# SandroMartens/DBGSOM

Measured on AMD Instinct MI355X. Metric: samples/sec/epoch (BMU+update), higher is better.
Workload: dtype f64; 1 GPU; Synthetic N=1e6 d=784 fp32, M=1024 (32x32); samples_total=1000000, samples_per_gpu=1000000, features=784, prototypes=1024, x_storage=f32, map=frozen (same prototypes every step), bmu_algorithm=filtered, via=HipBackend -> dbgsom_ctx_epoch (one C-ABI call per step)

## Files before the change

dbgsom_amd/backend.py:

```python
from __future__ import annotations

import ctypes
import os
from dataclasses import dataclass
from typing import Optional

import numpy as np

from . import _native


@dataclass
class EpochResult:
    new_weights: np.ndarray
    change_total: float
    errors: np.ndarray
    activations: np.ndarray
    winners: Optional[np.ndarray] = None
    distances: Optional[np.ndarray] = None
    new_weights_dev: object = None
    class_hist: Optional[np.ndarray] = None


def shard_bounds(n: int, rank: int, world: int):
# ... 293 lines not shown
                         lambda self, a: self._set("algorithm", _native.ALGORITHMS[a]))
    sweep_planes = property(lambda self: self._get("sweep_planes"),
                            lambda self, v: self._set("sweep_planes", v))
    seed_stride = property(lambda self: self._get("seed_stride"),
                           lambda self, v: self._set("seed_stride", v))
    refine = property(lambda self: self._get("refine"), lambda self, v: self._set("refine", int(v)))
    refined = property(lambda self: bool(self._get("refined")))
    defer = property(lambda self: bool(self._get("defer")), lambda self, v: self._set("defer", int(bool(v))))
    shard_smooth = property(lambda self: self._get("shard_smooth"), lambda self, v: self._set("shard_smooth", int(v)))
    shard_epochs = property(lambda self: self._get("shard_epochs"))
    defer_epochs = property(lambda self: self._get("defer_epochs"))
    csr_densify_below = property(lambda self: self._get("csr_densify_below"),
                                 lambda self, v: self._set("csr_densify_below", int(v)))
    resident_csr = property(lambda self: bool(self._get("resident_csr")))
    planes_cached = property(lambda self: bool(self._get("planes_cached")))
    padded_features = property(lambda self: self._get("padded_features"))

    @property
    def n_samples(self):
        return self._get("n_samples")

    def _require_loaded(self):
        if not self._loaded:
            raise RuntimeError("HipBackend: call load(X) first")

    def _install_collective(self):
        rank, world = dist_info()
        force = os.environ.get("DBGSOM_FORCE_COLLECTIVE") == "1" and _group_is_up()
        if world == 1 and not force:
            _native.call("dbgsom_ctx_set_collectives", self._ctx, None, None, 0, 1)
# ... 517 lines not shown
        keep, p, M, rf = self._w_arg(W)
        counts = np.empty(M, dtype=np.int64)
        win = np.empty(self._N, dtype=np.int64) if want_winners else None
        self._call("dbgsom_ctx_partition", self._ctx, p, M, rf, counts.ctypes.data,
                   None if win is None else win.ctypes.data)
        return counts, win

    def subset(self, neuron):
        child = ctypes.c_void_p()
        self._call("dbgsom_ctx_subset_create", self._ctx, int(neuron), ctypes.byref(child))
        sub = HipBackend(self.device_index, self.algorithm, _ctx=child)
        sub._weighted = self._weighted
        return sub

    _SETTABLE = ("algorithm", "sweep_planes", "seed_stride", "timing", "graph", "refine", "defer",
                 "filter_min_query_rows", "max_mean_candidates", "shard_smooth", "csr_densify_below")

    def release(self):
        if self._ctx:
            opts = {k: self._get(k) for k in self._SETTABLE}
            _native.call("dbgsom_ctx_destroy", self._ctx)
            self._ctx = ctypes.c_void_p()
            _native.call("dbgsom_ctx_create", self.device_index, ctypes.byref(self._ctx))
            for k, v in opts.items():
                self._set(k, v)
            self._install_collective()
        self._loaded = False
        self._borrowed = None
        self._hop_key = None
        self._weighted = False
        self._sw = None
# ... 9 lines not shown
```

dbgsom_amd/csrc/common.h:

```cpp
#pragma once
#include <hip/hip_runtime.h>
#include <stdint.h>
#include <stdio.h>

#include "../../include/dbgsom_hip.h"

namespace dbgsom {

void set_error(const char *fmt, ...);

#define DBGSOM_HIP_CHECK(expr)                                                           \
    do {                                                                                 \
        hipError_t _e = (expr);                                                          \
        if (_e != hipSuccess) {                                                          \
            ::dbgsom::set_error("%s failed: %s (%s:%d)", #expr, hipGetErrorString(_e),   \
                                __FILE__, __LINE__);                                     \
            return DBGSOM_EHIP;                                                          \
        }                                                                                \
    } while (0)

#define DBGSOM_REQUIRE(cond, msg)                                   \
    do {                                                            \
        if (!(cond)) {                                              \
            ::dbgsom::set_error("%s: %s", __func__, msg);           \
// ... 176 lines not shown
    const int32_t *order = nullptr;
    int seed_stride = 0, sweep_planes = 0, round_f32 = 0;
    int k = 1;
    int64_t *idx = nullptr;
    double *dist = nullptr;
    void *ws = nullptr;
    size_t ws_bytes = 0;
    hipStream_t stream = nullptr;
    const double *hint_dist = nullptr, *hint_shift = nullptr;
    int refine_rows = 0;
    bool defer_dist = false;
    const void *X_store = nullptr;
    int store_dtype = -1;
    int64_t ld_store = 0;
    double guard_mean = 0.0;
    FilterAux *aux = nullptr;
};
constexpr int DBGSOM_LISTS_LONG = 1000;
int launch_bmu_filtered(const FilteredCall &call);
size_t smooth_workspace_bytes(int64_t M, int64_t d);
int launch_smooth(const double *sums, int64_t M, int64_t d, const float *hop, double sigma,
                  int layout, const double *W_old, double *W_new, double *change_total, void *ws,
                  size_t ws_bytes, hipStream_t s);
int64_t smooth_block_cols(int64_t d, int nranks);
int64_t smooth_block_elems(int64_t M, int64_t d, int nranks);
int launch_pack_blocks(const double *sums, int64_t M, int64_t d, int nranks, double *out, hipStream_t s);
int launch_smooth_block(const double *S_b, const double *K, const double *a, int64_t M, int64_t cb, int64_t d_full,
                        const float *hop, double sigma, int layout, double *Wb, void *ws, size_t ws_bytes,
                        hipStream_t s);
int launch_rowchange_blocks(const double *blocks, int64_t M, int64_t d, int64_t cb, const double *W_old, double *W_new,
// ... 4 lines not shown
```

dbgsom_amd/csrc/engine.hip:

```cpp
#include <dlfcn.h>
#include <math.h>
#include <stdlib.h>
#include <string.h>

#include <chrono>
#include <new>
#include <vector>

#include "common.h"
#include "search_policy.h"

namespace dbgsom {

struct DevBuf {
    void *p = nullptr;
    size_t cap = 0;
    bool tight = false;
    int reserve(size_t bytes) {
        if (bytes <= cap) return DBGSOM_OK;
        if (p) { (void)hipFree(p); p = nullptr; cap = 0; }
        const size_t want = tight ? align_up(bytes) : align_up(bytes + bytes / 8, 1 << 20);
        hipError_t e = hipMalloc(&p, want);
        if (e != hipSuccess) {
            p = nullptr;
// ... 119 lines not shown
        dst[i] = src[ids[first + i]];
}
__global__ void gather_i32_kernel(const int32_t *__restrict__ src, const int32_t *__restrict__ ids, int64_t first,
                                  int64_t n, int32_t *__restrict__ dst) {
    for (int64_t i = (int64_t)blockIdx.x * blockDim.x + threadIdx.x; i < n; i += (int64_t)gridDim.x * blockDim.x)
        dst[i] = src[ids[first + i]];
}
template <typename T>
__global__ void rows_to_f64_kernel(const T *__restrict__ src, int64_t ld, const int64_t *__restrict__ ids, int64_t n,
                                   int64_t cols, double *__restrict__ dst) {
    const int64_t r = blockIdx.x;
    if (r >= n) return;
    const T *s = src + ids[r] * ld;
    for (int64_t c = threadIdx.x; c < cols; c += blockDim.x) dst[r * cols + c] = widen(s[c]);
}
__global__ void seg_counts_kernel(const uint32_t *__restrict__ seg_start, int64_t M, int64_t N, int64_t *__restrict__ counts) {
    for (int64_t j = (int64_t)blockIdx.x * blockDim.x + threadIdx.x; j < M; j += (int64_t)gridDim.x * blockDim.x)
        counts[j] = (int64_t)((j + 1 < M ? seg_start[j + 1] : (uint32_t)N) - seg_start[j]);
}

static unsigned grid1d(int64_t n, int block = 256) {
    const int64_t nb = (n + block - 1) / block;
    return (unsigned)(nb < 1 ? 1 : (nb > 8192 ? 8192 : nb));
}

}

using namespace dbgsom;

extern "C" {
const unsigned long long *dbgsom_filter_count_sum_ptr(const void *workspace_dev, int64_t N, int64_t d, int64_t M);
size_t dbgsom_filter_planes_bytes(int64_t rows, int64_t d);
size_t dbgsom_bmu_filtered_workspace_bytes(int64_t N, int64_t d, int64_t M);
}

namespace {

struct Samples {
    int dtype = -1;
    int64_t N = 0, d = 0, dp = 0;
    const void *X = nullptr;
    const void *Xb = nullptr;
    int bdtype = -1;
    DevBuf own, x32, xx, planes;
    bool planes_ready = false;
    bool csr = false;
    int64_t nnz = 0;
    DevBuf indptr, indices, data;
    CsrView view() const { return CsrView{indptr.as<int64_t>(), indices.as<int32_t>(), data.p}; }
    void release() {
        own.release(); x32.release(); xx.release(); planes.release(); indptr.release(); indices.release(); data.release();
        planes_ready = false; csr = false; nnz = 0; dtype = -1; N = 0; X = Xb = nullptr;
    }
};

}

struct dbgsom_ctx {
    int device = 0;
    hipStream_t stream = nullptr;
    int timing = 0;
    int use_graph = 0;
    int defer = 0;
    bool last_deferred = false;
    int64_t defer_epochs = 0;
    int last_round_f32 = 0;
    bool last_refined = false;
// ... 40 lines not shown
    void *rccl_comm = nullptr;
    bool rccl_owned = false;
    dbgsom_collective_fn coll = nullptr;
    void *coll_user = nullptr;
    int coll_rank = 0, coll_nranks = 1;
    int shard_smooth = 2;
    bool sums_sharded = false;
    int64_t shard_epochs = 0;
    DevBuf shard_send, shard_gather;
    int64_t w_up_calls = 0, w_up_bytes = 0, w_down_calls = 0, w_down_bytes = 0, w_row_writes = 0, w_row_reads = 0;
    hipEvent_t ev[4] = {};
    bool ev_created = false, ev_valid = false;
    double filter_ms[5] = {0, 0, 0, 0, 0};
    bool filter_ms_valid = false;
    FilterAux faux;
};

namespace {

#define CTX_CHECK(c)                                                                 \
    do {                                                                             \
        if (!(c)) { set_error("%s: null context", __func__); return DBGSOM_EINVAL; } \
        DBGSOM_HIP_CHECK(hipSetDevice((c)->device));                                 \
    } while (0)
#define TRY(expr) do { int _rc = (expr); if (_rc != DBGSOM_OK) return _rc; } while (0)

inline int64_t pad16(int64_t d) { return (d + 15) / 16 * 16; }

int sync(dbgsom_ctx *c) {
    DBGSOM_HIP_CHECK(hipStreamSynchronize(c->stream));
// ... 26 lines not shown
    if (s.dtype == DBGSOM_BF16) {
        if (!x32_is_widened) {
            TRY(s.x32.reserve((size_t)s.N * s.dp * 4));
            hipLaunchKernelGGL(widen_bf16_kernel, dim3(grid1d(s.N * s.dp)), dim3(256), 0, c->stream,
                               (const uint16_t *)s.X, s.x32.as<float>(), s.N * s.dp);
            TRY(launch_status("widen_bf16_kernel"));
        }
        s.Xb = s.x32.p;
        s.bdtype = DBGSOM_F32;
    } else {
        s.Xb = s.X;
        s.bdtype = s.dtype;
    }
    TRY(s.xx.reserve((size_t)s.N * 8));
    TRY(launch_row_sqnorms(s.Xb, s.bdtype, s.N, s.dp, s.dp, s.xx.as<double>(), c->stream));
    s.planes_ready = false;
    return DBGSOM_OK;
}

int place_host_samples(dbgsom_ctx *c, Samples &s, const void *X_host, int x_dtype, int64_t N, int64_t d, int storage) {
    DBGSOM_REQUIRE(valid_dtype(x_dtype) && valid_dtype(storage), "dtype must be DBGSOM_F32/F64/BF16");
    DBGSOM_REQUIRE(X_host && N >= 1 && d >= 1 && N < 0x7fffffff, "bad samples");
    DBGSOM_REQUIRE(storage == x_dtype || (storage == DBGSOM_BF16 && x_dtype == DBGSOM_F32),
                   "storage must be the input dtype, or DBGSOM_BF16 for float32 input");
    const int64_t dp = pad16(d);
    s.N = N; s.d = d; s.dp = dp; s.dtype = storage;
    s.csr = false; s.nnz = 0;
    bool widened = false;
    if (storage == DBGSOM_BF16 && x_dtype == DBGSOM_F32) {
        TRY(s.x32.reserve((size_t)N * dp * 4));
        TRY(s.own.reserve((size_t)N * dp * 2));
// ... 8 lines not shown
        TRY(upload_padded(c, s.own.p, X_host, N, d, dp, es));
    }
    s.X = s.own.p;
    return finish_samples(c, s, widened);
}

int ensure_planes(dbgsom_ctx *c, Samples &s) {
    if (s.planes_ready) return DBGSOM_OK;
    const size_t nbytes = dbgsom_filter_planes_bytes(s.N, s.dp);
    TRY(s.planes.reserve(nbytes));
    TRY(dbgsom_filter_prepare(s.Xb, s.bdtype, s.N, s.dp, s.dp, s.planes.p, s.planes.cap, c->stream));
    s.planes_ready = true;
    return DBGSOM_OK;
}

bool filter_shape_ok(const Samples &s, int64_t M) { return SearchPolicy::shape_ok(M, s.N, s.dp); }

bool filter_applies(const dbgsom_ctx *c, int64_t M) {
    if (c->xs.csr) return false;
    return c->policy.filter_allowed() && filter_shape_ok(c->xs, M);
}

bool hint_applies(const dbgsom_ctx *c, int64_t M) { return c->policy.takes_hint() && c->hint_valid && c->hintM <= M; }

int stage_weights(dbgsom_ctx *c, const double *W_host, int64_t M, int64_t d, int64_t dp) {
    DBGSOM_REQUIRE(M >= 1 && M <= 0x7fffff00, "bad prototype count");
    if (W_host) {
        TRY(c->Wb[c->cur].reserve((size_t)M * dp * 8));
        TRY(upload_padded(c, c->Wb[c->cur].p, W_host, M, d, dp, 8));
        if (c->distW_buf == c->cur) c->dist_bound_valid = false;
// ... 17 lines not shown
    const SearchPolicy::Plan plan = c->policy.plan(M, s.N, s.dp, prev_idx != nullptr, may_probe, bound_usable);
    FilteredCall call;
    call.aux = &c->faux;
    if (plan.hint_bound) {
        TRY(c->shiftb.reserve((size_t)M * 8));
        const int64_t rows = c->distW_M < M ? c->distW_M : M;
        hipLaunchKernelGGL(row_shift_kernel, dim3((unsigned)M), dim3(64), 0, c->stream, W,
                           c->Wb[c->distW_buf].as<double>(), s.dp, s.dp, rows, M, c->shiftb.as<double>());
        TRY(launch_status("row_shift_kernel"));
        call.hint_dist = c->dist.as<double>();
        call.hint_shift = c->shiftb.as<double>();
    }
    call.X = s.Xb; call.x_dtype = s.bdtype; call.N = s.N; call.d = s.dp; call.ldx = s.dp;
    call.xx = s.xx.as<double>(); call.xplanes = s.planes.p; call.W = W; call.M = M; call.ww = c->ww.as<double>();
    call.prev_idx = prev_idx; call.order = order; call.seed_stride = plan.seed_stride; call.sweep_planes = plan.sweep_planes;
    call.round_f32 = round_f32; call.idx = idx; call.dist = dist; call.ws = ws.p; call.ws_bytes = ws.cap;
    call.stream = c->stream;
    call.refine_rows = plan.refine_rows;
    c->last_refined = plan.refine;
    call.defer_dist = plan.refine && allow_defer && c->defer && M < 0xffff &&
                      accumulate_can_fill_distances(s.dtype, s.dp);
    c->last_deferred = call.defer_dist;
    c->last_round_f32 = round_f32;
    if (s.dtype == DBGSOM_BF16) { call.X_store = s.X; call.store_dtype = DBGSOM_BF16; call.ld_store = s.dp; }
    call.guard_mean = plan.guard_mean;
    const int rc_f = launch_bmu_filtered(call);
    c->last_filter_M = M; c->last_filter_N = s.N; c->last_filter_d = s.dp; c->last_filter_ws = ws.p;
    if (rc_f == DBGSOM_LISTS_LONG) {
        c->policy.on_guarded();
        c->last_refined = false;
// ... 145 lines not shown
        DBGSOM_HIP_CHECK(hipMemcpyAsync(s.data.p, data_host, (size_t)nnz * es, hipMemcpyHostToDevice, c->stream));
    }
    if (d < densify_below) {
        TRY(s.own.reserve((size_t)N * dp * es));
        TRY(launch_csr_densify(s.view(), x_dtype, N, d, dp, s.own.p, c->stream));
        s.X = s.own.p;
        TRY(finish_samples(c, s, false));
        TRY(sync(c));
        s.indptr.release(); s.indices.release(); s.data.release();
        s.nnz = 0;
        return DBGSOM_OK;
    }
    s.csr = true;
    s.bdtype = x_dtype;
    s.own.release(); s.x32.release(); s.planes.release();
    s.planes_ready = false;
    TRY(s.xx.reserve((size_t)N * 8));
    return launch_csr_row_sqnorms(s.view(), x_dtype, N, s.xx.as<double>(), c->stream);
}

int csr_search(dbgsom_ctx *c, Samples &s, const double *W, const double *ww, DevBuf &wt, int64_t M, int k, int round_f32,
               int64_t *idx, double *dist) {
    const int64_t ldwt = csr_wt_ld(M);
    TRY(wt.reserve((size_t)s.dp * ldwt * 8));
    TRY(launch_transpose_weights(W, M, s.dp, s.dp, wt.as<double>(), ldwt, c->stream));
    return launch_bmu_csr(s.view(), s.dtype, s.N, s.xx.as<double>(), wt.as<double>(), ldwt, M, ww, k, round_f32, idx,
                          dist, c->stream);
}
int csr_search(dbgsom_ctx *c, Samples &s, const double *W, int64_t M, int k, int round_f32, int64_t *idx, double *dist) {
    return csr_search(c, s, W, c->ww.as<double>(), c->wt, M, k, round_f32, idx, dist);
}
// ... 304 lines not shown
    } else if (!strcmp(name, "sc_chunk_rows")) {
        DBGSOM_REQUIRE(v >= 1 && v <= ((int64_t)1 << 22), "sc_chunk_rows must be in [1, 2^22]");
        c->sc_chunk_rows = v;
    } else if (!strcmp(name, "masked_chunk_rows")) {
        DBGSOM_REQUIRE(v >= 1 && v <= ((int64_t)1 << 22), "masked_chunk_rows must be in [1, 2^22]");
        c->masked_chunk_rows = v;
    } else if (!strcmp(name, "sc_cap")) {
        DBGSOM_REQUIRE(v >= 0 && v <= 64, "sc_cap must be in [0, 64] (0 = the library's cap)");
        c->sc_cap = v;
    } else if (!strcmp(name, "max_mean_candidates")) {
        DBGSOM_REQUIRE(v >= 1, "max_mean_candidates must be >= 1");
        c->policy.max_mean_candidates = v;
    } else if (!strcmp(name, "csr_densify_below")) {
        DBGSOM_REQUIRE(v >= 0, "csr_densify_below must be >= 0 (0 = CSR input always stays CSR)");
        c->csr_densify_below = v;
    } else {
        set_error("dbgsom_ctx_set_option: unknown option '%s'", name);
        return DBGSOM_EINVAL;
    }
    return DBGSOM_OK;
}

int dbgsom_ctx_get_option(dbgsom_ctx *c, const char *name, int64_t *v) {
    CTX_CHECK(c);
    DBGSOM_REQUIRE(name && v, "null pointer");
    if (!strcmp(name, "algorithm")) *v = c->policy.algorithm;
    else if (!strcmp(name, "sweep_planes")) *v = c->policy.sweep_planes;
    else if (!strcmp(name, "seed_stride")) *v = c->policy.seed_stride;
    else if (!strcmp(name, "timing")) *v = c->timing;
    else if (!strcmp(name, "graph")) *v = c->use_graph;
// ... 9 lines not shown
    else if (!strcmp(name, "k2_filtered")) *v = c->last_k2_filtered ? 1 : 0;
    else if (!strcmp(name, "filter_min_query_rows")) *v = c->filter_min_query_rows;
    else if (!strcmp(name, "max_mean_candidates")) *v = c->policy.max_mean_candidates;
    else if (!strcmp(name, "sc_chunk_rows")) *v = c->sc_chunk_rows;
    else if (!strcmp(name, "sc_cap")) *v = c->sc_cap;
    else if (!strcmp(name, "masked_chunk_rows")) *v = c->masked_chunk_rows;
    else if (!strcmp(name, "csr_densify_below")) *v = c->csr_densify_below;
    else if (!strcmp(name, "resident_csr")) *v = (c->xs.dtype >= 0 && c->xs.csr) ? 1 : 0;
    else if (!strcmp(name, "resident_nnz")) *v = (c->xs.dtype >= 0 && c->xs.csr) ? c->xs.nnz : 0;
    else if (!strcmp(name, "n_samples")) *v = c->xs.dtype < 0 ? 0 : c->xs.N;
    else if (!strcmp(name, "features")) *v = c->xs.dtype < 0 ? 0 : c->xs.d;
    else if (!strcmp(name, "padded_features")) *v = c->xs.dtype < 0 ? 0 : c->xs.dp;
    else if (!strcmp(name, "storage")) *v = c->xs.dtype;
    else if (!strcmp(name, "prototypes")) *v = c->M;
    else if (!strcmp(name, "planes_cached")) *v = c->xs.planes_ready ? 1 : 0;
    else if (!strcmp(name, "planes_used")) *v = c->policy.planes_used;
    else if (!strcmp(name, "planes_next")) *v = c->policy.planes_for_call();
    else if (!strcmp(name, "hint_valid")) *v = c->hint_valid ? 1 : 0;
    else if (!strcmp(name, "filter_backoff")) *v = c->policy.filter_backoff;
    else if (!strcmp(name, "plane_hold")) *v = c->policy.plane_hold;
    else if (!strcmp(name, "seed_mode")) *v = c->policy.seed_mode;
    else if (!strcmp(name, "prune_retry")) *v = c->policy.prune_retry ? 1 : 0;
    else if (!strcmp(name, "w_upload_calls")) *v = c->w_up_calls;
    else if (!strcmp(name, "w_upload_bytes")) *v = c->w_up_bytes;
    else if (!strcmp(name, "w_download_calls")) *v = c->w_down_calls;
    else if (!strcmp(name, "w_download_bytes")) *v = c->w_down_bytes;
    else if (!strcmp(name, "w_row_writes")) *v = c->w_row_writes;
    else if (!strcmp(name, "w_row_reads")) *v = c->w_row_reads;
    else if (!strcmp(name, "device_bytes")) {
        size_t tot = 0;
        for (const Samples *q : {&c->xs, &c->xq})
            tot += q->own.cap + q->x32.cap + q->xx.cap + q->planes.cap + q->indptr.cap + q->indices.cap + q->data.cap;
        DevBuf *bufs[] = CTX_DEVBUFS(c);
        for (DevBuf *b : bufs) tot += b->cap;
        *v = (int64_t)tot;
    } else {
        set_error("dbgsom_ctx_get_option: unknown option '%s'", name);
        return DBGSOM_EINVAL;
    }
    return DBGSOM_OK;
}

int dbgsom_ctx_stream(dbgsom_ctx *c, void **stream) {
    CTX_CHECK(c);
    DBGSOM_REQUIRE(stream, "null pointer");
    *stream = (void *)c->stream;
    return DBGSOM_OK;
}

static void set_tight(dbgsom_ctx *c, bool tight) {
    DevBuf *bufs[] = CTX_DEVBUFS(c);
    for (DevBuf *b : bufs) b->tight = tight;
    for (Samples *q : {&c->xs, &c->xq})
        for (DevBuf *b : {&q->own, &q->x32, &q->xx, &q->planes, &q->indptr, &q->indices, &q->data}) b->tight = tight;
}

static void reset_training_state(dbgsom_ctx *c) {
    c->hint_valid = c->last_idx_valid = c->part_valid = false;
    c->has_labels = false;
    c->has_weights = false;
    c->policy.reset();
    c->dist_bound_valid = false;
    c->last_filtered = false;
    c->sumsM = 0;
    c->M = c->otherM = 0;
}

int dbgsom_ctx_load(dbgsom_ctx *c, const void *X_host, int x_dtype, int64_t N, int64_t d, int storage) {
    CTX_CHECK(c);
    reset_training_state(c);
    set_tight(c, false);
    c->xs.dtype = -1;
    c->xs.indptr.release(); c->xs.indices.release(); c->xs.data.release();
    const int rc = place_host_samples(c, c->xs, X_host, x_dtype, N, d, storage);
    if (rc != DBGSOM_OK) { (void)hipStreamSynchronize(c->stream); c->xs.dtype = -1; return rc; }
    return sync(c);
// ... 553 lines not shown
    CTX_CHECK(c);
    TRY(loaded(c, __func__));
    DBGSOM_REQUIRE(change_total_host && errors_host && activations_host, "null output");
    DBGSOM_REQUIRE(layout == DBGSOM_CENTRES_COMPACT || layout == DBGSOM_CENTRES_ALIGNED, "bad layout");
    if (c->topoM != M) {
        set_error("dbgsom_ctx_epoch: topology holds %lld neurons, weights %lld (call "
                  "dbgsom_ctx_set_topology after growth)", (long long)c->topoM, (long long)M);
        return DBGSOM_ESTATE;
    }
    Samples &s = c->xs;
    int rc = DBGSOM_OK;
    do {
        if ((rc = stage_weights(c, W_host, M, s.d, s.dp))) break;
        mark(c, 0);
        const auto t_begin = std::chrono::steady_clock::now();
        if ((rc = epoch_bmu(c, M, round_f32))) break;
        mark(c, 1);
        const int measuring = c->policy.take_timing_form();
        const int64_t *idx = c->idx[c->icur].as<int64_t>();
        if ((rc = accumulate_and_reduce(c, idx, nullptr, gamma, c->dist.as<double>(), M))) break;
        c->hint_valid = true;
        c->hintM = M;
        mark(c, 2);
        rc = smooth_and_fetch(c, M, sigma, layout, flags, W_new_host, change_total_host, errors_host, activations_host,
                              idx, idx_host, dist_host);
        if (rc != DBGSOM_OK && rc != DBGSOM_ERANGE) break;
        SearchPolicy &pol = c->policy;
        if (measuring >= 0)
            pol.refine_timed(measuring, std::chrono::duration<double, std::milli>(std::chrono::steady_clock::now() - t_begin).count());
        if (c->last_filtered) {
            const bool clean = !pol.last_probed && !pol.last_guarded && measuring < 0 && !W_new_host && !idx_host && !dist_host;
            const double epoch_ms =
                clean ? std::chrono::duration<double, std::milli>(std::chrono::steady_clock::now() - t_begin).count() : NAN;
            const double *counted = c->tail.as<double>() + 2 * M + 2;
            pol.observe(counted[0], counted[1], counted[2], (s.N + 127) / 128, M, s.dp, (flags & DBGSOM_EPOCH_FROZEN) != 0,
                        epoch_ms);
        } else {
            pol.observe_unfiltered();
        }
    } while (0);
    if (rc != DBGSOM_OK && rc != DBGSOM_ERANGE) { (void)hipStreamSynchronize(c->stream); c->hint_valid = false; }
    return rc;
}

int dbgsom_ctx_update(dbgsom_ctx *c, const double *W_host, int64_t M, const int64_t *idx_host, const double *kw_host,
                      const double *dist_host, double sigma, int layout, double *W_new_host,
                      double *change_total_host, double *errors_host, double *activations_host) {
    CTX_CHECK(c);
    TRY(loaded(c, __func__));
    DBGSOM_REQUIRE(idx_host && kw_host && dist_host && change_total_host && errors_host && activations_host, "null pointer");
    DBGSOM_REQUIRE(layout == DBGSOM_CENTRES_COMPACT || layout == DBGSOM_CENTRES_ALIGNED, "bad layout");
// ... 378 lines not shown
```

dbgsom_amd/csrc/filter.hip:

```cpp
#include <math.h>
#include <type_traits>

#include "bmu_common.h"
#include "filter_form.h"

namespace dbgsom {

constexpr double FQ = 8323072.0;
constexpr double F16 = 32512.0;
constexpr int FNT = 512;
constexpr int FSTAGES = 3;
constexpr int SCHED_BINS = 16;
constexpr int SCHED_RETRY = 2 * SCHED_BINS + 10;
constexpr int SCHED_CTR = 2 * SCHED_BINS + 12;
constexpr int SCHED_SUM = 2 * SCHED_BINS + 6;
constexpr int RF_CTR = 4;
static_assert(SCHED_CTR % 2 == 0, "the 64-bit counters of the refinement sit behind the schedule's");

__device__ __forceinline__ double plane16_residual(double r2, double s, double amax, int d) {
    (void)s;
    return sqrt(r2) * (1.0 + 1e-9 + 2.3e-16 * (double)d) + sqrt((double)d) * amax * 4e-16;
}

template <typename T>
// ... 1491 lines not shown
        if (lane == 0) {
            if (retry_mode == 1 && base > retry_above) {
                retry_groups[atomicAdd(retry_len, 1ull)] = (int32_t)group;
            } else {
                if (retry_mode == 0 && base > retry_above) atomicAdd(retry_len, 1ull);
                if (!count_only) {
                    ucount[group] = base;
                    atomicAdd(&sched_ctr[sched_bin(base)], 1u);
                }
                atomicAdd(sum_out, (unsigned long long)base);
            }
        }
    }
}

constexpr int QUAD_MAX = 3;
constexpr int split_ring_stages(int jtl, int xs) {
    const int n = (40 * 1024) / (64 * 16 * xs + jtl * 16 * 16 * 8);
    return n > 6 ? 6 : (n < 3 ? 3 : n);
}
template <typename XT, int JTL, int SPLIT, int NS>
constexpr int subset_exact_lds_bytes() { return NS * ((128 / SPLIT) * KT * (int)sizeof(XT) + 16 * JTL * KT * 8); }

template <typename XT, int JTL, int NWV, int SPLIT = 1, int K = 1, int NS = 3>
__device__ __forceinline__ void subset_exact_workgroup(
    char *__restrict__ smem, const unsigned block,
    const XT *__restrict__ X, int64_t N, int d, int64_t ldx, const double *__restrict__ xx,
    const double *__restrict__ W, int M, const double *__restrict__ ww,
    const int32_t *__restrict__ order, const uint16_t *__restrict__ ulist, int ulist_stride,
    const uint32_t *__restrict__ ucount, const int32_t *__restrict__ sched,
// ... 367 lines not shown
    double *wres16;
    double *ctab, *yypad, *ctab_sub, *yy_sub, *ictab, *yctab, *yy_part, *summary;
    float *tab32;
    float *chk32;
    double *tile_score;
    double *tile_part;
    int32_t *kt_sel;
    uint16_t *ulist;
    uint32_t *ucount;
    int32_t *sched;
    uint32_t *sched_ctr;
    int64_t *seed;
    int32_t *order;
    float *gap;
    int32_t *retry;
    uint32_t *nnub;
    unsigned long long *cand;
    int64_t *rbest;
    int32_t *order2;
    int32_t *ovf;
    uint16_t *ovf_cand;
    uint8_t *gflag;
    unsigned long long *rf_ctr;
    uint32_t *rf_qlen;
    int32_t *rf_queue;
    int64_t Mg;
    void *sort_ws;
    int64_t nb, Mpad;
};
static size_t carve_filter(FilterWs *out, char *base, int64_t N, int64_t d, int64_t M) {
// ... 16 lines not shown
    take(f.tab32, (size_t)6 * Mpad * 4); take(f.chk32, (size_t)(Mpad / 256) * 16);
    take(f.tile_part, (size_t)TS_RB * 2 * dpad * 8);
    take(f.ulist, (size_t)nb * Mpad * 2); take(f.ucount, (size_t)nb * 4);
    take(f.seed, (size_t)N * 8); take(f.order, (size_t)N * 4);
    take(f.sort_ws, bucket_sort_workspace_bytes(N, M + 1));
    take(f.sched, (size_t)nb * 4); take(f.sched_ctr, (size_t)(SCHED_CTR + 2 * RF_CTR + 4) * 4);
    f.rf_ctr = base ? reinterpret_cast<unsigned long long *>(f.sched_ctr + SCHED_CTR) : nullptr;
    f.rf_qlen = base ? f.sched_ctr + SCHED_CTR + 2 * RF_CTR : nullptr;
    take(f.rf_queue, (size_t)2 * nb * 4);
    take(f.rbest, (size_t)N * 8); take(f.order2, (size_t)N * 4); take(f.ovf, (size_t)N * 8);
    take(f.cand, (size_t)N * 8); take(f.gflag, (size_t)nb);
    take(f.ovf_cand, (size_t)(N < OV_CAP ? N : OV_CAP) * OV_REC * 2);
    take(f.gap, M <= PRUNE_MAX_M ? (size_t)Mg * Mg * 4 : 0);
    if (M > PRUNE_MAX_M) f.gap = nullptr;
    take(f.retry, (size_t)nb * 4); take(f.nnub, (size_t)Mg * 4);
    f.Mg = Mg; f.nb = nb; f.Mpad = Mpad;
    return off;
}

static int launch_slice(const void *A, int dtype, int64_t rows, int64_t d, int64_t ld,
                        const PlaneBuf &b, hipStream_t s) {
    const int dpad = (int)filter_dpad(d);
    dim3 grid((unsigned)((rows + 3) / 4)), block(256);
    if (dtype == DBGSOM_F32)
        hipLaunchKernelGGL(slice_rows_kernel<float>, grid, block, 0, s, (const float *)A, rows, (int)d, ld, dpad, b.planes, b.scale, b.l1, b.res16);
    else if (dtype == DBGSOM_F64)
        hipLaunchKernelGGL(slice_rows_kernel<double>, grid, block, 0, s, (const double *)A, rows, (int)d, ld, dpad, b.planes, b.scale, b.l1, b.res16);
    else
        hipLaunchKernelGGL(slice_rows_kernel<bf16_t>, grid, block, 0, s, (const bf16_t *)A, rows, (int)d, ld, dpad, b.planes, b.scale, b.l1, b.res16);
    return launch_status("slice_rows_kernel");
// ... 117 lines not shown
                           hint ? c.hint_shift : nullptr, f.retry, retry_len(), retry_mode,
                           (uint32_t)(c.M / 8 > 96 ? c.M / 8 : 96), fm.k2 ? f.nnub : nullptr);
    }

    int gaps(hipStream_t gs) const {
        const unsigned gt = (unsigned)(f.Mg / 64);
        uint32_t *nnub = fm.k2 ? f.nnub : nullptr;
        if (nnub) DBGSOM_HIP_CHECK(hipMemsetAsync(nnub, 0x7f, (size_t)f.Mg * 4, gs));
        hipLaunchKernelGGL(fm.gap_nb == 2 ? proto_gap_kernel<2> : proto_gap_kernel<1>,
                           fm.gap_nb == 2 ? dim3(gt, gt) : dim3(2 * gt, 2 * gt), dim3(64), 0, gs, f.wt, (int)f.Mpad, dpad,
                           (int)c.M, d, f.wscale, f.wn0, c.ww, f.gap, (int)f.Mg, nnub);
        return DBGSOM_OK;
    }

    void prepare_prototypes() const {
        const bool select = fm.nkt_used < fm.nkt_full;
        if (select) {
            hipLaunchKernelGGL(tile_partial_kernel, dim3((unsigned)fm.nkt_full, TS_RB), dim3(256), 0, s, c.W, (int)c.M, d,
                               dpad, f.tile_part);
            hipLaunchKernelGGL(tile_score_select_kernel, dim3((unsigned)fm.nkt_full), dim3(64), 0, s, f.tile_part, (int)c.M,
                               dpad, f.tile_score, fm.nkt_full, fm.nkt_used, f.kt_sel, f.tickets + 0);
        }
        WTables tables;
        tables.ww = c.ww; tables.ctab = f.ctab; tables.yypad = f.yypad; tables.ctab_sub = f.ctab_sub;
        tables.yy_sub = f.yy_sub; tables.ictab = f.ictab; tables.yctab = f.yctab; tables.summary = f.summary;
        tables.sched_ctr = f.sched_ctr; tables.tscale = sweep_tscale(fm.sweep_planes); tables.tab32 = f.tab32; tables.chk32 = f.chk32;
        hipLaunchKernelGGL(slice_w_tiled_kernel, dim3((unsigned)((c.M + 3) / 4)), dim3(256), 0, s, c.W, (int)c.M, d, dpad,
                           (int)f.Mpad, fm.seed_stride, fm.Msubpad, fm.nkt_used, select ? f.kt_sel : (const int32_t *)nullptr,
                           f.wt, f.wt_sub, f.wscale, f.wl1, f.yy_part, f.wn0, f.wres16, f.tickets + 1, tables);
    }

    int seed_and_sort() {
        if (seeds) {
            aux.timer.mark(2, s);
            return DBGSOM_OK;
        }
        SideStream &side = aux.side;
        if (fm.gap_nb && side.ready()) {
            DBGSOM_HIP_CHECK(hipEventRecord(side.gap_fork, s));
            DBGSOM_HIP_CHECK(hipStreamWaitEvent(side.stream, side.gap_fork, 0));
            const int rc = gaps(side.stream);
            if (rc != DBGSOM_OK) return rc;
            DBGSOM_HIP_CHECK(hipEventRecord(side.gap_done, side.stream));
            gap_aside = true;
        }
        if (fm.sweep_planes == 1) sweep4(PREPASS);
        else sweep_i8(sweep_i8_kernel<1, 2, 2>, true);
        aux.timer.mark(2, s);
        seeds = f.seed;
        order = f.order;
        return launch_bucket_sort(f.seed, c.N, c.M, f.order, f.sort_ws, s);
    }

    int mark_candidates() const {
        if (fm.gap_nb) {
            if (gap_aside) {
                DBGSOM_HIP_CHECK(hipStreamWaitEvent(s, aux.side.gap_done, 0));
            } else {
                const int rc = gaps(s);
                if (rc != DBGSOM_OK) return rc;
            }
            prune_mark(fm.prune_retry ? 1 : 0, true);
            if (fm.prune_retry) {
                sweep4(RESEED);
                prune_mark(2, false);
            }
// ... 108 lines not shown
        }
        return DBGSOM_OK;
    }
};
}

int dbgsom::launch_bmu_filtered(const FilteredCall &call) {
    FilterForm form;
    const char *rejected = form.resolve(call.seed_stride, call.sweep_planes, call.k, call.refine_rows, call.defer_dist, call.N,
                                        call.d, call.M, call.prev_idx != nullptr);
    DBGSOM_REQUIRE(!rejected, rejected);
    DBGSOM_REQUIRE(call.x_dtype == DBGSOM_F32 || call.x_dtype == DBGSOM_F64, "the filtered search takes float32 or float64 samples");
    DBGSOM_REQUIRE(call.N >= 1 && call.N < 0x7fffffff && call.d >= 1 && call.d % KT == 0 && call.ldx >= call.d,
                   "bad sample shape (d must be a multiple of 16)");
    DBGSOM_REQUIRE(call.M >= 1 && call.M <= SW_MAX_M, "M outside [1, 16000]");
    DBGSOM_REQUIRE(call.X && call.xx && call.xplanes && call.W && call.ww && call.idx && call.dist && call.ws, "null pointer");
    DBGSOM_REQUIRE((call.prev_idx == nullptr) == (call.order == nullptr),
                   "prev_idx and order come as a pair (both NULL = stateless two-pass search)");
    DBGSOM_REQUIRE(is_aligned(call.X, 16) && (call.ldx * (int64_t)dtype_size(call.x_dtype)) % 16 == 0 &&
                       is_aligned(call.W, 16) && is_aligned(call.ws, 256) && is_aligned(call.xplanes, 256), "alignment");
    if (call.ws_bytes < dbgsom_bmu_filtered_workspace_bytes(call.N, call.d, call.M)) {
        set_error("dbgsom_bmu_filtered: workspace too small");
        return DBGSOM_ENOMEM;
    }
    FilterAux &aux = call.aux ? *call.aux : g_aux;
    FilterRun r{call, form, aux, call.stream, (int)call.d, (int)filter_dpad(call.d), {}, {}, call.prev_idx, call.order};
    carve_planes(&r.xb, (char *)const_cast<void *>(call.xplanes), call.N, call.d);
    carve_filter(&r.f, (char *)call.ws, call.N, call.d, call.M);
    StageTimer &timer = aux.timer;
    timer.mark(0, r.s);
    r.prepare_prototypes();
    timer.mark(1, r.s);
    int rc = r.seed_and_sort();
    if (rc != DBGSOM_OK) return rc;
    timer.mark(3, r.s);
    rc = r.mark_candidates();
    if (rc != DBGSOM_OK) return rc;
    timer.mark(4, r.s);
    rc = call.guard_mean > 0.0 ? r.guard_lists() : DBGSOM_OK;
    if (rc == DBGSOM_OK) rc = r.exact_on_candidates();
    if (rc != DBGSOM_OK && rc != DBGSOM_LISTS_LONG) return rc;
    timer.mark(5, r.s);
    timer.valid = timer.enabled;
    return rc == DBGSOM_LISTS_LONG ? rc : launch_status("filtered bmu kernels");
}

extern "C" {


// ... 49 lines not shown
```

Before: 460.6 million samples/s/epoch.

## Seed filtered BMU search from cached anchor clusters instead of per-sample sweep

Adds an anchor-based seeding path. 256 sample rows are chosen and ordered into a greedy nearest-neighbour chain, every sample is assigned to its nearest anchor once (cached, together with a bucket order), and each later epoch only computes anchor-to-prototype nearest seeds with a small MFMA f64 kernel, then gathers them per sample. This replaces the per-sample seed sweep and bucket sort on stateless pruning calls. The cost is a one-time anchor build, a fixed sample order that no longer follows the current winners, and possibly weaker seeds and more candidates. A heuristic drops the anchors when the mean candidate count rises above 1.25x the reference.

Result: faster. 500.2 million samples/s/epoch, median of 6 (+8.6%).

```diff
diff --git a/dbgsom_amd/backend.py b/dbgsom_amd/backend.py
--- a/dbgsom_amd/backend.py
+++ b/dbgsom_amd/backend.py
@@ -331,6 +331,10 @@
                                  lambda self, v: self._set("csr_densify_below", int(v)))
     resident_csr = property(lambda self: bool(self._get("resident_csr")))
     planes_cached = property(lambda self: bool(self._get("planes_cached")))
+    anchor_seeds = property(lambda self: self._get("anchor_seeds"), lambda self, v: self._set("anchor_seeds", int(v)))
+    anchor_builds = property(lambda self: self._get("anchor_builds"))
+    anchor_searches = property(lambda self: self._get("anchor_searches"))
+    anchor_state = property(lambda self: self._get("anchor_state"))
     padded_features = property(lambda self: self._get("padded_features"))
 
     @property
@@ -878,7 +882,7 @@
         return sub
 
     _SETTABLE = ("algorithm", "sweep_planes", "seed_stride", "timing", "graph", "refine", "defer",
-                 "filter_min_query_rows", "max_mean_candidates", "shard_smooth", "csr_densify_below")
+                 "filter_min_query_rows", "max_mean_candidates", "shard_smooth", "csr_densify_below", "anchor_seeds")
 
     def release(self):
         if self._ctx:
diff --git a/dbgsom_amd/csrc/common.h b/dbgsom_amd/csrc/common.h
--- a/dbgsom_amd/csrc/common.h
+++ b/dbgsom_amd/csrc/common.h
@@ -214,6 +214,10 @@
     int store_dtype = -1;
     int64_t ld_store = 0;
     double guard_mean = 0.0;
+    const double *anchors = nullptr;
+    const int32_t *anchor_of = nullptr;
+    int n_anchors = 0;
+    int32_t *seeds_out = nullptr, *order_out = nullptr;
     FilterAux *aux = nullptr;
 };
 constexpr int DBGSOM_LISTS_LONG = 1000;
diff --git a/dbgsom_amd/csrc/engine.hip b/dbgsom_amd/csrc/engine.hip
--- a/dbgsom_amd/csrc/engine.hip
+++ b/dbgsom_amd/csrc/engine.hip
@@ -157,6 +157,10 @@
     const T *s = src + ids[r] * ld;
     for (int64_t c = threadIdx.x; c < cols; c += blockDim.x) dst[r * cols + c] = widen(s[c]);
 }
+__global__ void iota_i32_kernel(int32_t *__restrict__ a, int32_t *__restrict__ b, int64_t n) {
+    for (int64_t i = (int64_t)blockIdx.x * blockDim.x + threadIdx.x; i < n; i += (int64_t)gridDim.x * blockDim.x)
+        a[i] = b[i] = (int32_t)i;
+}
 __global__ void seg_counts_kernel(const uint32_t *__restrict__ seg_start, int64_t M, int64_t N, int64_t *__restrict__ counts) {
     for (int64_t j = (int64_t)blockIdx.x * blockDim.x + threadIdx.x; j < M; j += (int64_t)gridDim.x * blockDim.x)
         counts[j] = (int64_t)((j + 1 < M ? seg_start[j + 1] : (uint32_t)N) - seg_start[j]);
@@ -187,13 +191,21 @@
     int bdtype = -1;
     DevBuf own, x32, xx, planes;
     bool planes_ready = false;
+    DevBuf anchors, anchor_of, anchor_order;
+    int64_t n_anchors = 0;
+    int anchor_state = 0;
+    void drop_anchors(int state) {
+        anchors.release(); anchor_of.release(); anchor_order.release();
+        n_anchors = 0; anchor_state = state;
+    }
+    void drop_planes() { planes_ready = false; drop_anchors(0); }
     bool csr = false;
     int64_t nnz = 0;
     DevBuf indptr, indices, data;
     CsrView view() const { return CsrView{indptr.as<int64_t>(), indices.as<int32_t>(), data.p}; }
     void release() {
         own.release(); x32.release(); xx.release(); planes.release(); indptr.release(); indices.release(); data.release();
-        planes_ready = false; csr = false; nnz = 0; dtype = -1; N = 0; X = Xb = nullptr;
+        drop_planes(); csr = false; nnz = 0; dtype = -1; N = 0; X = Xb = nullptr;
     }
 };
 
@@ -264,6 +276,12 @@
     double filter_ms[5] = {0, 0, 0, 0, 0};
     bool filter_ms_valid = false;
     FilterAux faux;
+    int anchor_seeds = 1;
+    int64_t anchor_builds = 0, anchor_searches = 0;
+    bool anchors_built_now = false;
+    bool last_anchor_seeded = false;
+    double prepass_mean = NAN;
+    int64_t prepass_M = 0;
 };
 
 namespace {
@@ -320,7 +338,7 @@
     }
     TRY(s.xx.reserve((size_t)s.N * 8));
     TRY(launch_row_sqnorms(s.Xb, s.bdtype, s.N, s.dp, s.dp, s.xx.as<double>(), c->stream));
-    s.planes_ready = false;
+    s.drop_planes();
     return DBGSOM_OK;
 }
 
@@ -359,6 +377,86 @@
     return DBGSOM_OK;
 }
 
+void chain_anchors(const std::vector<double> &a, int64_t A, int64_t dp, std::vector<int64_t> &rows) {
+    std::vector<double> d2((size_t)A * A, 0.0);
+    for (int64_t i = 0; i < A; ++i)
+        for (int64_t j = i + 1; j < A; ++j) {
+            const double *x = &a[(size_t)i * dp], *y = &a[(size_t)j * dp];
+            double acc = 0.0;
+            for (int64_t k = 0; k < dp; ++k) { const double t = x[k] - y[k]; acc += t * t; }
+            d2[(size_t)i * A + j] = d2[(size_t)j * A + i] = acc;
+        }
+    std::vector<char> taken((size_t)A, 0);
+    std::vector<int64_t> chain;
+    int64_t cur = 0;
+    for (int64_t n = 0; n < A; ++n) {
+        taken[(size_t)cur] = 1;
+        chain.push_back(rows[(size_t)cur]);
+        int64_t best = -1;
+        for (int64_t j = 0; j < A; ++j)
+            if (!taken[(size_t)j] && (best < 0 || d2[(size_t)cur * A + j] < d2[(size_t)cur * A + best])) best = j;
+        cur = best;
+    }
+    rows = chain;
+}
+
+int gather_anchor_rows(dbgsom_ctx *c, Samples &s, const std::vector<int64_t> &rows, double *anchors) {
+    const int64_t A = (int64_t)rows.size(), dp = s.dp;
+    TRY(c->stage_dev.reserve((size_t)A * 8));
+    int64_t *ids = c->stage_dev.as<int64_t>();
+    DBGSOM_HIP_CHECK(hipMemcpyAsync(ids, rows.data(), (size_t)A * 8, hipMemcpyHostToDevice, c->stream));
+    DBGSOM_HIP_CHECK(hipStreamSynchronize(c->stream));
+    if (s.dtype == DBGSOM_F32)
+        hipLaunchKernelGGL(rows_to_f64_kernel<float>, dim3((unsigned)A), dim3(256), 0, c->stream, (const float *)s.X, dp, ids, A, dp, anchors);
+    else if (s.dtype == DBGSOM_F64)
+        hipLaunchKernelGGL(rows_to_f64_kernel<double>, dim3((unsigned)A), dim3(256), 0, c->stream, (const double *)s.X, dp, ids, A, dp, anchors);
+    else
+        hipLaunchKernelGGL(rows_to_f64_kernel<bf16_t>, dim3((unsigned)A), dim3(256), 0, c->stream, (const bf16_t *)s.X, dp, ids, A, dp, anchors);
+    TRY(launch_status("rows_to_f64_kernel"));
+    return DBGSOM_OK;
+}
+
+int ensure_anchors(dbgsom_ctx *c, Samples &s) {
+    if (s.anchor_state != 0) return DBGSOM_OK;
+    TRY(ensure_planes(c, s));
+    const int64_t A = s.N < 256 ? s.N : 256, dp = s.dp;
+    TRY(s.anchors.reserve((size_t)A * dp * 8 + (size_t)A * 8));
+    TRY(s.anchor_of.reserve((size_t)s.N * 4));
+    TRY(s.anchor_order.reserve((size_t)s.N * 4));
+    std::vector<int64_t> rows((size_t)A);
+    for (int64_t k = 0; k < A; ++k) rows[(size_t)k] = k * s.N / A;
+    double *anchors = s.anchors.as<double>(), *anorm = anchors + (size_t)A * dp;
+    TRY(gather_anchor_rows(c, s, rows, anchors));
+    if (A < s.N && A > 2) {
+        std::vector<double> host((size_t)A * dp);
+        DBGSOM_HIP_CHECK(hipMemcpyAsync(host.data(), anchors, (size_t)A * dp * 8, hipMemcpyDeviceToHost, c->stream));
+        DBGSOM_HIP_CHECK(hipStreamSynchronize(c->stream));
+        chain_anchors(host, A, dp, rows);
+        TRY(gather_anchor_rows(c, s, rows, anchors));
+    }
+    if (A == s.N) {
+        hipLaunchKernelGGL(iota_i32_kernel, dim3(grid1d(s.N)), dim3(256), 0, c->stream, s.anchor_of.as<int32_t>(),
+                           s.anchor_order.as<int32_t>(), s.N);
+        TRY(launch_status("iota_i32_kernel"));
+    } else {
+        TRY(launch_row_sqnorms(anchors, DBGSOM_F64, A, dp, dp, anorm, c->stream));
+        TRY(c->filt_ws.reserve_zeroed(dbgsom_bmu_filtered_workspace_bytes(s.N, dp, A), c->stream));
+        FilteredCall call;
+        call.aux = &c->faux;
+        call.X = s.Xb; call.x_dtype = s.bdtype; call.N = s.N; call.d = dp; call.ldx = dp;
+        call.xx = s.xx.as<double>(); call.xplanes = s.planes.p; call.W = anchors; call.M = A; call.ww = anorm;
+        call.seed_stride = DBGSOM_SEED_FULL; call.sweep_planes = 1;
+        call.seeds_out = s.anchor_of.as<int32_t>(); call.order_out = s.anchor_order.as<int32_t>();
+        call.ws = c->filt_ws.p; call.ws_bytes = c->filt_ws.cap; call.stream = c->stream;
+        TRY(launch_bmu_filtered(call));
+    }
+    s.n_anchors = A;
+    s.anchor_state = 1;
+    ++c->anchor_builds;
+    c->anchors_built_now = true;
+    return DBGSOM_OK;
+}
+
 bool filter_shape_ok(const Samples &s, int64_t M) { return SearchPolicy::shape_ok(M, s.N, s.dp); }
 
 bool filter_applies(const dbgsom_ctx *c, int64_t M) {
@@ -406,6 +504,16 @@
     call.X = s.Xb; call.x_dtype = s.bdtype; call.N = s.N; call.d = s.dp; call.ldx = s.dp;
     call.xx = s.xx.as<double>(); call.xplanes = s.planes.p; call.W = W; call.M = M; call.ww = c->ww.as<double>();
     call.prev_idx = prev_idx; call.order = order; call.seed_stride = plan.seed_stride; call.sweep_planes = plan.sweep_planes;
+    c->last_anchor_seeded = false;
+    const bool has_ref = c->prepass_mean == c->prepass_mean && SearchPolicy::near_size(M, c->prepass_M);
+    if (!prev_idx && &s == &c->xs && c->anchor_seeds && s.anchor_state != 2 && has_ref && plan.planes == 0 &&
+        !plan.seed_full && (plan.seed_stride & DBGSOM_PRUNE)) {
+        TRY(ensure_anchors(c, s));
+        ++c->anchor_searches;
+        call.anchors = s.anchors.as<double>(); call.n_anchors = (int)s.n_anchors;
+        call.anchor_of = s.anchor_of.as<int32_t>(); call.order = s.anchor_order.as<int32_t>();
+        c->last_anchor_seeded = true;
+    }
     call.round_f32 = round_f32; call.idx = idx; call.dist = dist; call.ws = ws.p; call.ws_bytes = ws.cap;
     call.stream = c->stream;
     call.refine_rows = plan.refine_rows;
@@ -581,7 +689,7 @@
     s.csr = true;
     s.bdtype = x_dtype;
     s.own.release(); s.x32.release(); s.planes.release();
-    s.planes_ready = false;
+    s.drop_planes();
     TRY(s.xx.reserve((size_t)N * 8));
     return launch_csr_row_sqnorms(s.view(), x_dtype, N, s.xx.as<double>(), c->stream);
 }
@@ -916,6 +1024,9 @@
     } else if (!strcmp(name, "csr_densify_below")) {
         DBGSOM_REQUIRE(v >= 0, "csr_densify_below must be >= 0 (0 = CSR input always stays CSR)");
         c->csr_densify_below = v;
+    } else if (!strcmp(name, "anchor_seeds")) {
+        DBGSOM_REQUIRE(v == 0 || v == 1, "anchor_seeds must be 0 or 1");
+        c->anchor_seeds = (int)v;
     } else {
         set_error("dbgsom_ctx_set_option: unknown option '%s'", name);
         return DBGSOM_EINVAL;
@@ -955,6 +1066,10 @@
     else if (!strcmp(name, "storage")) *v = c->xs.dtype;
     else if (!strcmp(name, "prototypes")) *v = c->M;
     else if (!strcmp(name, "planes_cached")) *v = c->xs.planes_ready ? 1 : 0;
+    else if (!strcmp(name, "anchor_seeds")) *v = c->anchor_seeds;
+    else if (!strcmp(name, "anchor_builds")) *v = c->anchor_builds;
+    else if (!strcmp(name, "anchor_searches")) *v = c->anchor_searches;
+    else if (!strcmp(name, "anchor_state")) *v = c->xs.dtype < 0 ? 0 : c->xs.anchor_state;
     else if (!strcmp(name, "planes_used")) *v = c->policy.planes_used;
     else if (!strcmp(name, "planes_next")) *v = c->policy.planes_for_call();
     else if (!strcmp(name, "hint_valid")) *v = c->hint_valid ? 1 : 0;
@@ -971,7 +1086,8 @@
     else if (!strcmp(name, "device_bytes")) {
         size_t tot = 0;
         for (const Samples *q : {&c->xs, &c->xq})
-            tot += q->own.cap + q->x32.cap + q->xx.cap + q->planes.cap + q->indptr.cap + q->indices.cap + q->data.cap;
+            tot += q->own.cap + q->x32.cap + q->xx.cap + q->planes.cap + q->indptr.cap + q->indices.cap + q->data.cap +
+                   q->anchors.cap + q->anchor_of.cap + q->anchor_order.cap;
         DevBuf *bufs[] = CTX_DEVBUFS(c);
         for (DevBuf *b : bufs) tot += b->cap;
         *v = (int64_t)tot;
@@ -993,7 +1109,9 @@
     DevBuf *bufs[] = CTX_DEVBUFS(c);
     for (DevBuf *b : bufs) b->tight = tight;
     for (Samples *q : {&c->xs, &c->xq})
-        for (DevBuf *b : {&q->own, &q->x32, &q->xx, &q->planes, &q->indptr, &q->indices, &q->data}) b->tight = tight;
+        for (DevBuf *b : {&q->own, &q->x32, &q->xx, &q->planes, &q->indptr, &q->indices, &q->data, &q->anchors, &q->anchor_of,
+                          &q->anchor_order})
+            b->tight = tight;
 }
 
 static void reset_training_state(dbgsom_ctx *c) {
@@ -1001,6 +1119,8 @@
     c->has_labels = false;
     c->has_weights = false;
     c->policy.reset();
+    c->prepass_mean = NAN;
+    c->last_anchor_seeded = false;
     c->dist_bound_valid = false;
     c->last_filtered = false;
     c->sumsM = 0;
@@ -1584,6 +1704,7 @@
         if ((rc = stage_weights(c, W_host, M, s.d, s.dp))) break;
         mark(c, 0);
         const auto t_begin = std::chrono::steady_clock::now();
+        c->anchors_built_now = false;
         if ((rc = epoch_bmu(c, M, round_f32))) break;
         mark(c, 1);
         const int measuring = c->policy.take_timing_form();
@@ -1599,12 +1720,27 @@
         if (measuring >= 0)
             pol.refine_timed(measuring, std::chrono::duration<double, std::milli>(std::chrono::steady_clock::now() - t_begin).count());
         if (c->last_filtered) {
-            const bool clean = !pol.last_probed && !pol.last_guarded && measuring < 0 && !W_new_host && !idx_host && !dist_host;
+            const bool clean = !pol.last_probed && !pol.last_guarded && measuring < 0 && !W_new_host && !idx_host && !dist_host &&
+                               !c->anchors_built_now;
             const double epoch_ms =
                 clean ? std::chrono::duration<double, std::milli>(std::chrono::steady_clock::now() - t_begin).count() : NAN;
             const double *counted = c->tail.as<double>() + 2 * M + 2;
-            pol.observe(counted[0], counted[1], counted[2], (s.N + 127) / 128, M, s.dp, (flags & DBGSOM_EPOCH_FROZEN) != 0,
-                        epoch_ms);
+            const int64_t nb = (s.N + 127) / 128;
+            const bool settled = !(counted[2] > 0.0 && !pol.last_retry);
+            if (pol.last_probed && !pol.last_hinted && !pol.last_seed_full && settled) {
+                c->prepass_mean = counted[1] / (double)nb;
+                c->prepass_M = M;
+            }
+            if (pol.planes_used == 0 && !pol.last_hinted && !pol.last_seed_full && settled) {
+                const double mean = counted[0] / (double)nb;
+                if (c->last_anchor_seeded) {
+                    if (mean > 1.25 * c->prepass_mean) s.drop_anchors(2);
+                } else {
+                    c->prepass_mean = mean;
+                    c->prepass_M = M;
+                }
+            }
+            pol.observe(counted[0], counted[1], counted[2], nb, M, s.dp, (flags & DBGSOM_EPOCH_FROZEN) != 0, epoch_ms);
         } else {
             pol.observe_unfiltered();
         }
diff --git a/dbgsom_amd/csrc/filter.hip b/dbgsom_amd/csrc/filter.hip
--- a/dbgsom_amd/csrc/filter.hip
+++ b/dbgsom_amd/csrc/filter.hip
@@ -1529,6 +1529,89 @@
     }
 }
 
+typedef double ad4_t __attribute__((ext_vector_type(4)));
+constexpr int ANCHOR_MAX = 256;
+constexpr int ANCHOR_TICKET0 = 16;
+
+__device__ __forceinline__ bool seed_less(double v, int j, double bv, int bj) { return v < bv || (v == bv && j < bj); }
+
+__global__ __launch_bounds__(256) void anchor_seed_kernel(const double *__restrict__ anchors, int A,
+                                                          const double *__restrict__ W, int M, int d,
+                                                          const double *__restrict__ ww, double *__restrict__ part_val,
+                                                          int32_t *__restrict__ part_idx, uint32_t *__restrict__ tickets,
+                                                          int32_t *__restrict__ aseed) {
+    __shared__ double val_s[4][16];
+    __shared__ int idx_s[4][16];
+    const int tid = threadIdx.x, lane = tid & 63, wave = tid >> 6, r = lane & 15, q = lane >> 4;
+    const int npart = gridDim.x, ab = blockIdx.y * 16, jb = blockIdx.x * 64 + wave * 16;
+    const int jrow = min(jb + r, M - 1), arow = min(ab + r, A - 1);
+    const double *wp = W + (size_t)jrow * d + 4 * q, *ap = anchors + (size_t)arow * d + 4 * q;
+    ad4_t c = {0.0, 0.0, 0.0, 0.0};
+#pragma unroll 4
+    for (int k = 0; k < d; k += 16) {
+        const ad4_t wv = *reinterpret_cast<const ad4_t *>(wp + k), av = *reinterpret_cast<const ad4_t *>(ap + k);
+        c = __builtin_amdgcn_mfma_f64_16x16x4f64(wv[0], av[0], c, 0, 0, 0);
+        c = __builtin_amdgcn_mfma_f64_16x16x4f64(wv[1], av[1], c, 0, 0, 0);
+        c = __builtin_amdgcn_mfma_f64_16x16x4f64(wv[2], av[2], c, 0, 0, 0);
+        c = __builtin_amdgcn_mfma_f64_16x16x4f64(wv[3], av[3], c, 0, 0, 0);
+    }
+    double bv = INFINITY;
+    int bj = 0x7fffffff;
+#pragma unroll
+    for (int u = 0; u < 4; ++u) {
+        const int j = jb + 4 * u + q;
+        if (j >= M) continue;
+        const double y = ww[j], v = y - 2.0 * c[u];
+        const double key = fabs(y) < INFINITY ? (fabs(v) < INFINITY ? v : 1.7976931348623157e308) : INFINITY;
+        if (seed_less(key, j, bv, bj)) { bv = key; bj = j; }
+    }
+#pragma unroll
+    for (int off = 16; off < 64; off <<= 1) {
+        const double ov = __shfl_xor(bv, off, 64);
+        const int oj = __shfl_xor(bj, off, 64);
+        if (seed_less(ov, oj, bv, bj)) { bv = ov; bj = oj; }
+    }
+    if (q == 0) { val_s[wave][r] = bv; idx_s[wave][r] = bj; }
+    __syncthreads();
+    if (tid < 16 && ab + tid < A) {
+        bv = val_s[0][tid]; bj = idx_s[0][tid];
+#pragma unroll
+        for (int w = 1; w < 4; ++w)
+            if (seed_less(val_s[w][tid], idx_s[w][tid], bv, bj)) { bv = val_s[w][tid]; bj = idx_s[w][tid]; }
+        part_val[(size_t)(ab + tid) * npart + blockIdx.x] = bv;
+        part_idx[(size_t)(ab + tid) * npart + blockIdx.x] = bj;
+    }
+    if (!last_workgroup_done(tickets + ANCHOR_TICKET0 + blockIdx.y, (uint32_t)npart)) return;
+    const int a = ab + (tid >> 4), sub = tid & 15;
+    bv = INFINITY; bj = 0x7fffffff;
+    if (a < A)
+        for (int p = sub; p < npart; p += 16) {
+            const double v = part_val[(size_t)a * npart + p];
+            const int j = part_idx[(size_t)a * npart + p];
+            if (seed_less(v, j, bv, bj)) { bv = v; bj = j; }
+        }
+#pragma unroll
+    for (int off = 1; off < 16; off <<= 1) {
+        const double ov = __shfl_xor(bv, off, 64);
+        const int oj = __shfl_xor(bj, off, 64);
+        if (seed_less(ov, oj, bv, bj)) { bv = ov; bj = oj; }
+    }
+    if (sub == 0 && a < A) aseed[a] = bj;
+}
+
+__global__ __launch_bounds__(256) void anchor_gather_kernel(const int32_t *__restrict__ aseed,
+                                                            const int32_t *__restrict__ anchor_of, int64_t N,
+                                                            int64_t *__restrict__ seed) {
+    for (int64_t i = (int64_t)blockIdx.x * 256 + threadIdx.x; i < N; i += (int64_t)gridDim.x * 256)
+        seed[i] = (int64_t)aseed[anchor_of[i]];
+}
+
+__global__ __launch_bounds__(256) void narrow_seeds_kernel(const int64_t *__restrict__ seed, int64_t N,
+                                                           int32_t *__restrict__ out) {
+    for (int64_t i = (int64_t)blockIdx.x * 256 + threadIdx.x; i < N; i += (int64_t)gridDim.x * 256)
+        out[i] = (int32_t)seed[i];
+}
+
 constexpr int QUAD_MAX = 3;
 constexpr int split_ring_stages(int jtl, int xs) {
     const int n = (40 * 1024) / (64 * 16 * xs + jtl * 16 * 16 * 8);
@@ -1926,6 +2009,9 @@
     int32_t *order;
     float *gap;
     int32_t *retry;
+    int32_t *aseed;
+    double *apart_val;
+    int32_t *apart_idx;
     uint32_t *nnub;
     unsigned long long *cand;
     int64_t *rbest;
@@ -1972,6 +2058,8 @@
     take(f.gap, M <= PRUNE_MAX_M ? (size_t)Mg * Mg * 4 : 0);
     if (M > PRUNE_MAX_M) f.gap = nullptr;
     take(f.retry, (size_t)nb * 4); take(f.nnub, (size_t)Mg * 4);
+    take(f.aseed, (size_t)ANCHOR_MAX * 4);
+    take(f.apart_val, (size_t)ANCHOR_MAX * (Mg / 64) * 8); take(f.apart_idx, (size_t)ANCHOR_MAX * (Mg / 64) * 4);
     f.Mg = Mg; f.nb = nb; f.Mpad = Mpad;
     return off;
 }
@@ -2119,7 +2207,7 @@
     }
 
     void prepare_prototypes() const {
-        const bool select = fm.nkt_used < fm.nkt_full;
+        const bool select = fm.nkt_used < fm.nkt_full && !c.anchor_of;
         if (select) {
             hipLaunchKernelGGL(tile_partial_kernel, dim3((unsigned)fm.nkt_full, TS_RB), dim3(256), 0, s, c.W, (int)c.M, d,
                                dpad, f.tile_part);
@@ -2140,6 +2228,7 @@
             aux.timer.mark(2, s);
             return DBGSOM_OK;
         }
+        if (c.anchor_of) return seed_from_anchors();
         SideStream &side = aux.side;
         if (fm.gap_nb && side.ready()) {
             DBGSOM_HIP_CHECK(hipEventRecord(side.gap_fork, s));
@@ -2154,7 +2243,31 @@
         aux.timer.mark(2, s);
         seeds = f.seed;
         order = f.order;
+        if (c.seeds_out) {
+            hipLaunchKernelGGL(narrow_seeds_kernel, dim3(seed_grid()), dim3(256), 0, s, f.seed, c.N, c.seeds_out);
+            return launch_bucket_sort(f.seed, c.N, c.M, c.order_out, f.sort_ws, s);
+        }
         return launch_bucket_sort(f.seed, c.N, c.M, f.order, f.sort_ws, s);
+    }
+
+    unsigned seed_grid() const { const int64_t g = (c.N + 255) / 256; return (unsigned)(g < 2048 ? g : 2048); }
+
+    int seed_from_anchors() {
+        SideStream &side = aux.side;
+        if (fm.gap_nb && side.ready()) {
+            DBGSOM_HIP_CHECK(hipEventRecord(side.gap_fork, s));
+            DBGSOM_HIP_CHECK(hipStreamWaitEvent(side.stream, side.gap_fork, 0));
+            const int rc = gaps(side.stream);
+            if (rc != DBGSOM_OK) return rc;
+            DBGSOM_HIP_CHECK(hipEventRecord(side.gap_done, side.stream));
+            gap_aside = true;
+        }
+        hipLaunchKernelGGL(anchor_seed_kernel, dim3((unsigned)(f.Mg / 64), (unsigned)((c.n_anchors + 15) / 16)), dim3(256),
+                           0, s, c.anchors, c.n_anchors, c.W, (int)c.M, d, c.ww, f.apart_val, f.apart_idx, f.tickets, f.aseed);
+        hipLaunchKernelGGL(anchor_gather_kernel, dim3(seed_grid()), dim3(256), 0, s, f.aseed, c.anchor_of, c.N, f.seed);
+        aux.timer.mark(2, s);
+        seeds = f.seed;
+        return DBGSOM_OK;
     }
 
     int mark_candidates() const {
@@ -2293,8 +2406,15 @@
     DBGSOM_REQUIRE(call.N >= 1 && call.N < 0x7fffffff && call.d >= 1 && call.d % KT == 0 && call.ldx >= call.d,
                    "bad sample shape (d must be a multiple of 16)");
     DBGSOM_REQUIRE(call.M >= 1 && call.M <= SW_MAX_M, "M outside [1, 16000]");
-    DBGSOM_REQUIRE(call.X && call.xx && call.xplanes && call.W && call.ww && call.idx && call.dist && call.ws, "null pointer");
-    DBGSOM_REQUIRE((call.prev_idx == nullptr) == (call.order == nullptr),
+    const bool seeds_only = call.seeds_out != nullptr;
+    DBGSOM_REQUIRE(call.X && call.xx && call.xplanes && call.W && call.ww && call.ws, "null pointer");
+    DBGSOM_REQUIRE(seeds_only || (call.idx && call.dist), "null pointer");
+    DBGSOM_REQUIRE(!seeds_only || (call.order_out && !call.prev_idx && !call.anchor_of && call.k == 1),
+                   "seeds_out comes with order_out, on a stateless k = 1 call");
+    DBGSOM_REQUIRE(!call.anchor_of || (call.anchors && call.order && !call.prev_idx && call.n_anchors >= 1 &&
+                                       call.n_anchors <= ANCHOR_MAX && form.prune && !form.seed_full && call.k == 1),
+                   "anchor seeds: the stateless k = 1 pruning form, with the anchors and the bucket order");
+    DBGSOM_REQUIRE(call.anchor_of || (call.prev_idx == nullptr) == (call.order == nullptr),
                    "prev_idx and order come as a pair (both NULL = stateless two-pass search)");
     DBGSOM_REQUIRE(is_aligned(call.X, 16) && (call.ldx * (int64_t)dtype_size(call.x_dtype)) % 16 == 0 &&
                        is_aligned(call.W, 16) && is_aligned(call.ws, 256) && is_aligned(call.xplanes, 256), "alignment");
@@ -2312,6 +2432,7 @@
     timer.mark(1, r.s);
     int rc = r.seed_and_sort();
     if (rc != DBGSOM_OK) return rc;
+    if (seeds_only) return launch_status("seed pre-pass and bucket sort");
     timer.mark(3, r.s);
     rc = r.mark_candidates();
     if (rc != DBGSOM_OK) return rc;
```
